# cherise215/advchain

Measured on AMD Instinct MI355X. Metric: augmented images/sec (N adv steps, chain=noise+bias+morph+affine), higher is better.
Workload: dtype f32

## Files before the change

advchain_amd/_lib.py:

```python
import ctypes
import os
from ctypes import c_char_p, c_float, c_int, c_int64, c_void_p

_HERE = os.path.dirname(os.path.abspath(__file__))
LIB_PATH = os.path.join(_HERE, "csrc", "libadvchain_hip.so")

_P, _I, _L, _F = c_void_p, c_int, c_int64, c_float

PROTOTYPES = {
    "advchain_version": (_I, []),
    "advchain_last_error": (c_char_p, []),
    "advchain_set_deterministic": (None, [_I]),
    "advchain_get_deterministic": (_I, []),
    "advchain_grid_sample_fwd": (_I, [_P, _P, _P, _L, _L, _I, _P, _P, _I, _I, _I, _P]),
    "advchain_grid_sample_fwd_ride": (_I, [_P, _P, _P, _P, _P, _L, _L, _I, _P, _P, _I, _I, _I, _I, _P]),
    "advchain_scatter_workspace": (_L, [_L, _I, _P]),
    "advchain_grid_sample_bwd": (_I, [_P, _P, _P, _P, _P, _P, _L, _L, _I, _P, _P, _I, _I, _I, _I, _P]),
    "advchain_det_warp_workspace": (_L, [_L, _L, _I, _P]),
    "advchain_grid_sample_bwd_det": (_I, [_P, _P, _P, _P, _P, _P, _L, _L, _I, _P, _P, _I, _I, _I, _P]),
    "advchain_compose_self_fwd": (_I, [_P, _P, _P, _L, _I, _P, _I, _P, _P]),
    "advchain_compose_self_bwd": (_I, [_P, _P, _P, _P, _I, _I, _L, _I, _P, _P]),
    "advchain_affine_warp_fwd": (_I, [_P, _P, _P, _L, _L, _I, _P, _I, _I, _P]),
    "advchain_affine_warp_fwd_ride": (_I, [_P, _P, _P, _P, _P, _L, _L, _I, _P, _I, _I, _I, _P]),
    "advchain_affine_warp_bwd_workspace": (_L, [_L, _I, _P]),
    "advchain_affine_warp_bwd": (_I, [_P, _P, _P, _P, _P, _P, _L, _L, _I, _P, _I, _I, _P]),
    "advchain_affine_warp_bwd_det": (_I, [_P, _P, _P, _P, _P, _P, _P, _L, _L, _I, _P, _I, _I, _P]),
    "advchain_affine_theta_fwd": (_I, [_P, _P, _F, _P, _P, _L, _I, _P]),
    "advchain_affine_theta_bwd": (_I, [_P, _P, _F, _P, _P, _P, _L, _I, _P]),
    "advchain_tp_interp_fwd": (_I, [_P, _P, _P, _P, _P, _P, _P, _L, _L, _I, _I, _F, _P, _P, _P]),
    "advchain_tp_interp_fwd_smoothed_pair": (_I, [_P, _P, _P, _P, _P, _P, _P, _P, _L, _L, _I, _F, _P, _P, _F, _P]),
    "advchain_band_reduce_axis": (_I, [_P, _P, _P, _P, _P, _P, _P, _P, _I, _L, _L, _F, _P]),
    "advchain_band_reduce_rows_dense": (_I, [_P, _P, _P, _P, _P, _L, _L, _L, _L, _F, _P]),
    "advchain_bias_field_fwd": (_I, [_P, _P, _P, _P, _P, _P, _P, _P, _P, _L, _L, _F, _I, _F, _P]),
    "advchain_bias_field_bwd": (_I, [_P, _P, _P, _P, _P, _P, _P, _P, _P, _P, _L, _L, _F, _I, _F, _P]),
    "advchain_gauss_axis": (_I, [_P, _P, _P, _L, _L, _I, _P, _I, _P, _I, _I, _F, _P]),
    "advchain_gauss_axis_generic": (_I, [_P, _P, _L, _I, _P, _I, _P, _I, _F, _P]),
    "advchain_max_displacement": (_I, [_P, _P, _L, _I, _P, _P]),
    "advchain_grid_sample_bicubic2d_fwd": (_I, [_P, _P, _P, _L, _L, _P, _P, _I, _P]),
    "advchain_grid_sample_bicubic2d_bwd": (_I, [_P, _P, _P, _P, _P, _L, _L, _P, _P, _I, _P]),
    "advchain_affine_grid2d_fwd": (_I, [_P, _P, _L, _P, _P]),
# ... 163 lines not shown
```

advchain_amd/csrc/common.h:

```cpp
#pragma once
#include <hip/hip_runtime.h>
#include <stdint.h>

namespace advchain {

enum { INTERP_LINEAR = 0, INTERP_NEAREST = 1 };
enum { PAD_ZEROS = 0, PAD_BORDER = 1, PAD_REFLECTION = 2 };

constexpr int kBlock = 256;

struct Dims {
  int s0, s1, s2;
  __host__ __device__ int64_t voxels() const { return (int64_t)s0 * s1 * s2; }
};

__device__ __forceinline__ float mul_nc(float a, float b) {
#pragma clang fp contract(off)
  return a * b;
}

__device__ __forceinline__ float lin_coord(int i, int S) {
  if (S <= 1) return S == 1 ? -1.f : 0.f;
  const float step = 2.f / (float)(S - 1);
  return (i < S / 2) ? (-1.f + step * (float)i) : (1.f - step * (float)(S - 1 - i));
// ... 135 lines not shown
__device__ __forceinline__ float fix_out(float cell, const FixScale& s) { return __builtin_amdgcn_ldexpf(cell * s.inv, -s.shift); }
__device__ __forceinline__ bool fix_plain(const FixScale& s, float& scale, float& inv) {
  scale = __builtin_amdgcn_ldexpf(s.mul, s.shift);
  inv = __builtin_amdgcn_ldexpf(s.inv, -s.shift);
  return scale <= 3.40282347e38f && inv >= 1.17549435e-38f && inv <= 3.40282347e38f;
}
__device__ __forceinline__ float fix_out_add(float cell, float a, const FixScale& s) {
  return __builtin_amdgcn_ldexpf(fmaf(cell, s.inv, __builtin_amdgcn_ldexpf(a, s.shift)), -s.shift);
}

__device__ __forceinline__ void atomic_add_f32(float* p, float v) {
  unsafeAtomicAdd(p, v);
}

}

#define ADVCHAIN_OK 0
#define ADVCHAIN_ERR_ARG (-1)
#define ADVCHAIN_ERR_UNSUPPORTED (-2)
#define ADVCHAIN_ERR_LAUNCH (-3)

extern "C" void advchain_set_error_(const char* msg);

#define ADVCHAIN_CHECK_ARG(cond, msg)      \
  do {                                     \
    if (!(cond)) {                         \
      advchain_set_error_(msg);            \
      return ADVCHAIN_ERR_ARG;             \
    }                                      \
  } while (0)

#define ADVCHAIN_LAUNCH_CHECK()                          \
  do {                                                   \
    hipError_t e_ = hipGetLastError();                   \
    if (e_ != hipSuccess) {                              \
      advchain_set_error_(hipGetErrorString(e_));        \
      return ADVCHAIN_ERR_LAUNCH;                        \
    }                                                    \
  } while (0)

static inline int advchain_blocks(int64_t n, int per_block) { return (int)((n + per_block - 1) / per_block); }

static __global__ void __launch_bounds__(256) k_zero_fill(float* __restrict__ p, int64_t n) {
  const int64_t stride = (int64_t)gridDim.x * 256 * 4;
  for (int64_t i = ((int64_t)blockIdx.x * 256 + threadIdx.x) * 4; i < n; i += stride) {
    if (i + 4 <= n && ((uintptr_t)(p + i) & 15) == 0) {
// ... 14 lines not shown
```

advchain_amd/csrc/error.cpp:

```cpp
#include <string.h>

#include <atomic>

static thread_local char g_last_error[512] = "";

extern "C" void advchain_set_error_(const char* msg) {
  strncpy(g_last_error, msg ? msg : "", sizeof(g_last_error) - 1);
  g_last_error[sizeof(g_last_error) - 1] = 0;
}

extern "C" const char* advchain_last_error(void) { return g_last_error; }

static std::atomic<int> g_deterministic{0};
extern "C" void advchain_set_deterministic(int on) { g_deterministic.store(on ? 1 : 0, std::memory_order_relaxed); }
extern "C" int advchain_get_deterministic(void) { return g_deterministic.load(std::memory_order_relaxed); }

extern "C" int advchain_version(void) { return 180; }
```

advchain_amd/csrc/sampler.hip:

```cpp
#include <stdlib.h>
#include "sampler_common.h"
#include "affine_geo.h"
#include "det_fix.h"

namespace advchain {

template <int UNR>
__device__ __forceinline__ void load_str(const float* __restrict__ p, int n, float (&r)[UNR]) {
#pragma unroll
  for (int k = 0; k < UNR; ++k) r[k] = p[(k < n ? k : 0) * kBlock];
#pragma unroll
  for (int k = 0; k < UNR; ++k) r[k] = k < n ? r[k] : 0.f;
}
template <int UNR>
__device__ __forceinline__ void store_str(float* __restrict__ p, int n, const float (&r)[UNR]) {
#pragma unroll
  for (int k = 0; k < UNR; ++k)
    if (k < n) p[k * kBlock] = r[k];
}
__device__ __forceinline__ int active_count(int64_t v0, int64_t total, int unr) {
  if (v0 >= total) return 0;
  const int64_t left = (total - v0 + kBlock - 1) / kBlock;
  return left < unr ? (int)left : unr;
}
// ... 633 lines not shown
}

}

using namespace advchain;

int advchain_scatter_tiled_launch(bool self, const float* gout, const float* in, const float* grid, float* gin,
                                  float* ggrid, int64_t N, int64_t C, int ndim, Dims d, int padding, int clamp_grid,
                                  int32_t* workspace, int chain, int halo, hipStream_t st);

int advchain_self_adjoint_gather_launch(const float* gout, const float* phi, float* gphi, int64_t N, int ndim, Dims d,
                                        int32_t* workspace, int chain, int halo, hipStream_t st);

int advchain_warp_adjoint_gather_launch(const float* gout, const float* in, const float* grid, float* gin, float* ggrid,
                                        int64_t N, int64_t C, int ndim, Dims d, int padding, int clamp_grid,
                                        int32_t* workspace, int halo, hipStream_t st);

int advchain_scatter_march_launch(bool self, const float* gout, const float* in, const float* grid, float* gin, float* ggrid,
                                  int64_t N, int64_t C, Dims d, int padding, int clamp_grid, int H, int32_t* workspace,
                                  hipStream_t st);

int advchain_scatter_window_launch(bool self, const float* gout, const float* in, const float* grid, float* gin,
                                   float* ggrid, int64_t N, int64_t C, int ndim, Dims d, int padding, int clamp_grid,
                                   int halo, int32_t* workspace, hipStream_t st, int32_t* det_ws);
int advchain_scatter_rows2d_launch(bool self, const float* gout, const float* in, const float* grid, float* gin, float* ggrid,
                                   int64_t N, int64_t C, Dims d, int padding, int clamp_grid, int H, int32_t* workspace,
                                   hipStream_t st, int rm_flags = 0);
bool advchain_scatter_rows2d_takes(bool self, int64_t C, Dims d, int padding, int H, int64_t N);

bool advchain_affine_box_fwd_launch(const float* in, const float* theta, float* out, int64_t N, int64_t C, int ndim, Dims d,
                                    hipStream_t st, const float* ride_in = nullptr, float* ride_out = nullptr,
                                    int ride_nonzero = 0);
int advchain_affine_box_tiles(int ndim, Dims d);
int advchain_affine_box_gtheta_launch(const float* gout, const float* in, const float* theta, float* gpart, int64_t N,
                                      int64_t C, int ndim, Dims d, int max_blocks, hipStream_t st, float* tilemax, float* geo = nullptr, int* mode = nullptr);
bool advchain_affine_box_gin_launch(const float* gout, const float* theta, const float* geo, const int* mode, float* gin,
                                    int64_t N, int64_t C, int ndim, Dims d, hipStream_t st, const float* tilemax);

int advchain_expo_fused_fwd2d_launch(const float* phi0, float* fields, int64_t N, advchain::Dims d, int k, int halos,
                                     float* disp_rows, float* fail_flag, hipStream_t stream, bool query = false);
int advchain_adjoint_fused2d_launch(const float* gk, const float* phi0, const float* fields, float* g0, int64_t N, advchain::Dims d,
                                    int k, int32_t* workspace, hipStream_t st);
int advchain_sample_tiled_launch(bool self, const float* in, const float* grid, float* out, const float* phi0,
                                 int64_t N, int64_t C, int ndim, Dims d, int padding, int clamp_grid, int final_mode,
                                 int halo, float* disp_out, hipStream_t st, int disp_hint);

static inline bool use_unroll(int64_t voxels, int ndim) {
// ... 150 lines not shown
}

int advchain_grid_sample_fwd_ride(const float* in, const float* grid, float* out, const float* ride_in, float* ride_out,
                                  int64_t N, int64_t C, int ndim, const int64_t* in_dims, const int64_t* out_dims, int interp,
                                  int padding, int clamp_grid, int flags, void* stream) {
  ADVCHAIN_CHECK_ARG(ride_in && ride_out && ride_out != out, "grid_sample_fwd_ride: null/aliased rider");
  ADVCHAIN_CHECK_ARG((flags & ~1) == 0, "grid_sample_fwd_ride: unknown flags");
  if (ndim == 2 && in && grid && out && dims_ok(ndim, in_dims) && dims_ok(ndim, out_dims, 1) && N > 0 && N < 65536 && C >= 1 &&
      (interp == INTERP_LINEAR || interp == INTERP_NEAREST) && padding >= 0 && padding <= 2) {
    const Dims id = make_dims(ndim, in_dims), od = make_dims(ndim, out_dims);
    ADVCHAIN_CHECK_ARG(id.voxels() < (1ll << 31) && od.voxels() < (1ll << 31), "grid_sample_fwd_ride: per-sample volume too large");
    return launch_grid_sample_fwd<2>(in, grid, out, N, C, id, od, interp, padding, clamp_grid & 1, (hipStream_t)stream, ride_in,
                                     ride_out, flags & 1);
  }
  int rc = advchain_grid_sample_fwd(in, grid, out, N, C, ndim, in_dims, out_dims, interp, padding, clamp_grid, stream);
  if (rc != ADVCHAIN_OK) return rc;
  rc = advchain_grid_sample_fwd(ride_in, grid, ride_out, N, 1, ndim, in_dims, out_dims, interp, padding, clamp_grid, stream);
  if (rc != ADVCHAIN_OK || !(flags & 1) || N == 0) return rc;
  int64_t total = N;
  for (int a = 0; a < ndim; ++a) total *= out_dims[a];
  return advchain_nonzero_mask(ride_out, ride_out, total, stream);
}

int advchain_grid_sample_bwd(const float* grad_out, const float* in, const float* grid, float* grad_in,
                             float* grad_grid, int32_t* workspace, int64_t N, int64_t C, int ndim,
                             const int64_t* in_dims, const int64_t* out_dims, int interp, int padding, int clamp_grid,
                             int halo, void* stream) {
  ADVCHAIN_CHECK_ARG(grad_out && in && grid, "grid_sample_bwd: null pointer");
  ADVCHAIN_CHECK_ARG(grad_in || grad_grid, "grid_sample_bwd: nothing to compute");
  ADVCHAIN_CHECK_ARG(dims_ok(ndim, in_dims) && dims_ok(ndim, out_dims, 1), "grid_sample_bwd: bad dims");
  ADVCHAIN_CHECK_ARG(N >= 0 && N < 65536 && C >= 1, "grid_sample_bwd: bad N/C");
  ADVCHAIN_CHECK_ARG(interp == INTERP_LINEAR || interp == INTERP_NEAREST, "grid_sample_bwd: interp");
  ADVCHAIN_CHECK_ARG(padding >= 0 && padding <= 2, "grid_sample_bwd: padding");
  if (N == 0) return ADVCHAIN_OK;
  const Dims id = make_dims(ndim, in_dims), od = make_dims(ndim, out_dims);
  ADVCHAIN_CHECK_ARG(id.voxels() < (1ll << 31) && od.voxels() < (1ll << 31), "grid_sample_bwd: per-sample volume too large");
  const bool same = id.s0 == od.s0 && id.s1 == od.s1 && id.s2 == od.s2;
  if (workspace && grad_in && same && interp == INTERP_LINEAR && C <= 4) {
    if (ndim == 2 && halo <= -2) {
      const int rr = advchain_scatter_rows2d_launch(false, grad_out, in, grid, grad_in, grad_grid, N, C, id, padding, clamp_grid,
                                                    -halo, workspace, (hipStream_t)stream);
      if (rr != ADVCHAIN_ERR_UNSUPPORTED) return rr;
    }
    const int rc = advchain_warp_adjoint_gather_launch(grad_out, in, grid, grad_in, grad_grid, N, C, ndim, id, padding,
                                                       clamp_grid, workspace, halo, (hipStream_t)stream);
    if (rc != ADVCHAIN_ERR_UNSUPPORTED) return rc;
    if (ndim == 3 && halo <= -2) {
      const int rm = advchain_scatter_march_launch(false, grad_out, in, grid, grad_in, grad_grid, N, C, id, padding, clamp_grid,
                                                   -halo, workspace, (hipStream_t)stream);
      if (rm != ADVCHAIN_ERR_UNSUPPORTED) return rm;
    }
    const int rw = advchain_scatter_window_launch(false, grad_out, in, grid, grad_in, grad_grid, N, C, ndim, id, padding,
                                                  clamp_grid, halo, nullptr, (hipStream_t)stream, workspace);
    if (rw != ADVCHAIN_ERR_UNSUPPORTED) return rw;
    return advchain_scatter_tiled_launch(false, grad_out, in, grid, grad_in, grad_grid, N, C, ndim, id, padding,
                                         clamp_grid, workspace, 0, halo < 0 ? -halo : halo, (hipStream_t)stream);
  }
  if (workspace && grad_in) advchain_zero_async(grad_in, sizeof(float) * N * C * id.voxels(), (hipStream_t)stream);
  return ndim == 3 ? launch_grid_sample_bwd<3>(grad_out, in, grid, grad_in, grad_grid, N, C, id, od, interp, padding, clamp_grid, (hipStream_t)stream)
                   : launch_grid_sample_bwd<2>(grad_out, in, grid, grad_in, grad_grid, N, C, id, od, interp, padding, clamp_grid, (hipStream_t)stream);
}

int64_t advchain_det_warp_workspace(int64_t N, int64_t C, int ndim, const int64_t* in_dims) {
  if (!in_dims || !dims_ok(ndim, in_dims, 1) || N < 0 || C < 1) return -1;
  return det_warp_image_ints(N, C, make_dims(ndim, in_dims).voxels()) + ((N + 3) & ~(int64_t)3);
}

int advchain_grid_sample_bwd_det(const float* grad_out, const float* in, const float* grid, float* grad_in,
                                 float* grad_grid, int32_t* det_ws, int64_t N, int64_t C, int ndim,
                                 const int64_t* in_dims, const int64_t* out_dims, int interp, int padding, int clamp_grid,
                                 void* stream) {
  ADVCHAIN_CHECK_ARG(grad_out && in && grid, "grid_sample_bwd_det: null pointer");
  ADVCHAIN_CHECK_ARG(grad_in || grad_grid, "grid_sample_bwd_det: nothing to compute");
  ADVCHAIN_CHECK_ARG(!grad_in || det_ws, "grid_sample_bwd_det: det_ws required for grad_in (advchain_det_warp_workspace int32 elements)");
  ADVCHAIN_CHECK_ARG(in_dims && out_dims && dims_ok(ndim, in_dims) && dims_ok(ndim, out_dims, 1), "grid_sample_bwd_det: bad dims");
  ADVCHAIN_CHECK_ARG(N >= 0 && N < 65536 && C >= 1, "grid_sample_bwd_det: bad N/C");
  ADVCHAIN_CHECK_ARG(interp == INTERP_LINEAR || interp == INTERP_NEAREST, "grid_sample_bwd_det: interp");
  ADVCHAIN_CHECK_ARG(padding >= 0 && padding <= 2, "grid_sample_bwd_det: padding");
  if (N == 0) return ADVCHAIN_OK;
  const Dims id = make_dims(ndim, in_dims), od = make_dims(ndim, out_dims);
  ADVCHAIN_CHECK_ARG(id.voxels() < (1ll << 31) && od.voxels() < (1ll << 31), "grid_sample_bwd_det: per-sample volume too large");
  hipStream_t st = (hipStream_t)stream;
  clamp_grid &= 1;
// ... 455 lines not shown
```

advchain_amd/csrc/scatter_window.hip:

```cpp
#include <stdlib.h>
#include "sampler_common.h"
#include "det_fix.h"

namespace advchain {

template <bool DET>
__device__ __forceinline__ void win_global_add(float* __restrict__ gin, unsigned long long* __restrict__ acc, int64_t idx,
                                               float v, const FixScale& sdet) {
  if (DET) atomicAdd(acc + idx, (unsigned long long)__float2ll_rn(fix_in(v * sdet.mul, sdet)));
  else atomic_add_f32(gin + idx, v);
}
#ifndef ADVCHAIN_WINDOW_FLAT
#define ADVCHAIN_WINDOW_FLAT 1
#endif
constexpr int kWinT = 32;
constexpr int kWinCells = 8192;
constexpr int kWinCellsC4 = 12288;

template <int PAD, int C, bool SELF, bool GG, bool DET = false>
__global__ void __launch_bounds__(kBlock)
k_scatter_window2d(const float* __restrict__ gout, const float* __restrict__ in, const float* __restrict__ grid,
                   float* __restrict__ gin, float* __restrict__ ggrid, Dims d, int n2, int clamp_grid,
                   int32_t* __restrict__ ws, unsigned long long* __restrict__ acc64 = nullptr,
                   const float* __restrict__ maxn = nullptr) {
  constexpr int kCells2 = C == 4 ? kWinCellsC4 : kWinCells;
  __shared__ int win[kCells2];
  if (ws && blockIdx.x == 0 && blockIdx.y == 0 && threadIdx.x == 0) ws[3] = -1;
  __shared__ int red[8][kBlock / 64];
  constexpr int DIM = 2;
  constexpr int SPT = kWinT * kWinT / kBlock;
  const int V = (int)d.voxels();
  const int n = blockIdx.y;
  const int tx = blockIdx.x % n2, ty = blockIdx.x / n2;
  const int lx = threadIdx.x & 31, ly0 = threadIdx.x >> 5;
  const int sx = tx * kWinT + lx;
  const float* gn = grid + (int64_t)n * DIM * V;
  const float* gon = gout + (int64_t)n * C * V;
  const float* inn = in + (int64_t)n * C * V;
  float* ginn = gin + (int64_t)n * C * V;
  unsigned long long* accn = DET ? acc64 + (int64_t)n * C * V : nullptr;
  const FixScale sdet = DET ? det_scale(maxn, n) : FixScale{0, 0.f, 0.f};

  Taps<DIM, PAD> t[SPT];
  float go[SPT][C];
  bool live[SPT], px[SPT], py[SPT];
  int bx0 = 1 << 30, bx1 = -(1 << 30), by0 = 1 << 30, by1 = -(1 << 30);
  float gmax = 0.f;
#pragma unroll
  for (int j = 0; j < SPT; ++j) {
    const int sy = ty * kWinT + ly0 + 8 * j;
    live[j] = sx < d.s2 && sy < d.s1;
    const int s = live[j] ? sy * d.s2 + sx : 0;
    float gx = gn[s], gy = gn[V + s];
    px[j] = py[j] = true;
    if (clamp_grid) {
      px[j] = gx >= -1.f && gx <= 1.f; py[j] = gy >= -1.f && gy <= 1.f;
      gx = clamp_unit(gx); gy = clamp_unit(gy);
    }
    t[j].build(gx, gy, 0.f, d);
#pragma unroll
    for (int c = 0; c < C; ++c) {
      const float g = gon[(int64_t)c * V + s];
      go[j][c] = live[j] ? g : 0.f;
      gmax = fmaxf(gmax, fabsf(go[j][c]));
    }
    if (live[j]) {
      if (t[j].x.v0 || t[j].x.v1) { bx0 = min(bx0, t[j].x.i0 + (t[j].x.v0 ? 0 : 1)); bx1 = max(bx1, t[j].x.i0 + (t[j].x.v1 ? 1 : 0)); }
      if (t[j].y.v0 || t[j].y.v1) { by0 = min(by0, t[j].y.i0 + (t[j].y.v0 ? 0 : 1)); by1 = max(by1, t[j].y.i0 + (t[j].y.v1 ? 1 : 0)); }
    }
  }
#pragma unroll
  for (int o = 32; o > 0; o >>= 1) {
    bx0 = min(bx0, __shfl_xor(bx0, o, 64)); bx1 = max(bx1, __shfl_xor(bx1, o, 64));
    by0 = min(by0, __shfl_xor(by0, o, 64)); by1 = max(by1, __shfl_xor(by1, o, 64));
    gmax = fmaxf(gmax, __shfl_xor(gmax, o, 64));
  }
  const int wave = threadIdx.x >> 6;
  if ((threadIdx.x & 63) == 0) {
    red[0][wave] = bx0; red[1][wave] = bx1; red[2][wave] = by0; red[3][wave] = by1; red[4][wave] = __float_as_int(gmax);
  }
  __syncthreads();
#pragma unroll
  for (int w = 0; w < kBlock / 64; ++w) {
    bx0 = min(bx0, red[0][w]); bx1 = max(bx1, red[1][w]); by0 = min(by0, red[2][w]); by1 = max(by1, red[3][w]);
    gmax = fmaxf(gmax, __int_as_float(red[4][w]));
  }
  int ww = max(bx1 - bx0 + 1, 0), wh = max(by1 - by0 + 1, 0);
  constexpr int cells_per_ch = kCells2 / C;
  if (ww > 128) ww = 128;
  if (ww > 0 && wh > cells_per_ch / ww) wh = cells_per_ch / ww;
  const int cells = ww * wh;
  for (int i = threadIdx.x; i < C * cells; i += kBlock) win[i] = 0;
  const FixScale fs = fix_scale(gmax, 20);
  __syncthreads();

  float cgx[SPT], cgy[SPT];
  if (SELF || GG) {
#pragma unroll
    for (int j = 0; j < SPT; ++j) {
      float ax = 0.f, ay = 0.f, dummy = 0.f;
#pragma unroll
      for (int c = 0; c < C; ++c)
        sample_linear_bwd<DIM, PAD, false, true>(inn + (int64_t)c * V, nullptr, go[j][c], t[j], d, ax, ay, dummy);
      cgx[j] = px[j] ? t[j].x.mult * ax : 0.f;
      cgy[j] = py[j] ? t[j].y.mult * ay : 0.f;
    }
  }

#pragma unroll
  for (int j = 0; j < SPT; ++j) {
    if (!live[j]) continue;
    const int sy = ty * kWinT + ly0 + 8 * j;
    const int s = sy * d.s2 + sx;
    const int wx0 = t[j].x.i0 - bx0, wy0 = t[j].y.i0 - by0;
    const int cell0 = __mul24(wy0, ww) + wx0;
    const int vox0 = __mul24(t[j].y.i0, d.s2) + t[j].x.i0;
    const bool inx[2] = {wx0 >= 0 && wx0 < ww, wx0 + 1 >= 0 && wx0 + 1 < ww};
    const bool iny[2] = {wy0 >= 0 && wy0 < wh, wy0 + 1 >= 0 && wy0 + 1 < wh};
#pragma unroll
    for (int cy = 0; cy < 2; ++cy)
#pragma unroll
      for (int cx = 0; cx < 2; ++cx) {
        if (!t[j].ok(0, cy, cx)) continue;
        const float w = t[j].w(0, cy, cx);
        if (inx[cx] && iny[cy]) {
          const float ws = w * fs.mul;
          int* cell = win + cell0 + (cy ? ww : 0) + cx;
#pragma unroll
          for (int c = 0; c < C; ++c) atomicAdd(cell + c * cells, fix_round(ws * fix_in(go[j][c], fs)));
        } else {
          const int64_t dst = vox0 + (cy ? d.s2 : 0) + cx;
#pragma unroll
          for (int c = 0; c < C; ++c) win_global_add<DET>(ginn, accn, dst + (int64_t)c * V, w * go[j][c], sdet);
        }
      }
    if (SELF || GG) {
      const float ggx = cgx[j], ggy = cgy[j];
      if (SELF) {
        if (ggx != 0.f) win_global_add<DET>(ginn, accn, s, ggx, sdet);
        if (ggy != 0.f) win_global_add<DET>(ginn, accn, (int64_t)V + s, ggy, sdet);
      } else {
        float* gg = ggrid + (int64_t)n * DIM * V + s;
        gg[0] = ggx;
        gg[V] = ggy;
      }
    }
  }
  __syncthreads();

  for (int i = threadIdx.x; i < C * cells; i += kBlock) {
    const int a = win[i];
    if (a == 0) continue;
    const int c = i / cells, r = i - c * cells;
    const int wy = r / ww, wx = r - wy * ww;
    win_global_add<DET>(ginn, accn, (int64_t)c * V + (by0 + wy) * d.s2 + (bx0 + wx), fix_out((float)a, fs), sdet);
  }
}

#ifndef ADVCHAIN_WIN3_CP4
#define ADVCHAIN_WIN3_CP4 2
#endif
#ifndef ADVCHAIN_WIN3_CPS
#define ADVCHAIN_WIN3_CPS 3
#endif
constexpr int kWin3CP4 = ADVCHAIN_WIN3_CP4, kWin3CPS = ADVCHAIN_WIN3_CPS;
constexpr int kWin3Cells = 12288;

template <int PAD, int C, bool SELF, bool GG, int TX, int TZ, bool DET = false>
__global__ void __launch_bounds__(kBlock)
k_scatter_window3d(const float* __restrict__ gout, const float* __restrict__ in, const float* __restrict__ grid,
                   float* __restrict__ gin, float* __restrict__ ggrid, Dims d, int n1, int n2, int clamp_grid,
                   int32_t* __restrict__ ws, unsigned long long* __restrict__ acc64 = nullptr,
                   const float* __restrict__ maxn = nullptr) {
  __shared__ int win[kWin3Cells];
  constexpr int CP = C == 4 ? kWin3CP4 : (SELF ? kWin3CPS : C);
  if (ws && blockIdx.x == 0 && blockIdx.y == 0 && threadIdx.x == 0) ws[3] = -1;
  __shared__ int red[7][kBlock / 64];
  constexpr int DIM = 3;
// ... 184 lines not shown
  {
    const float inv_ww = 1.f / (float)max(ww, 1), inv_wh = 1.f / (float)max(wh, 1), inv_wd = 1.f / (float)max(wd, 1);
    for (int i = threadIdx.x; i < CP * cells; i += kBlock) {
      const int a = win[i];
      if (a == 0) continue;
      const int r = (int)(((float)i + 0.5f) * inv_ww), wx = i - r * ww;
      const int rz = (int)(((float)r + 0.5f) * inv_wh), wy = r - rz * wh;
      const int c = (int)(((float)rz + 0.5f) * inv_wd), wz = rz - c * wd;
      win_global_add<DET>(ginn, accn, (int64_t)(c0 + c) * V + ((lo[2] + wz) * d.s1 + (lo[1] + wy)) * d.s2 + (lo[0] + wx),
                          fix_out((float)a, fs), sdet);
    }
  }
  if (c0 + CP < C) __syncthreads();
  }
}

}

using namespace advchain;

extern "C" int advchain_get_deterministic(void);
int advchain_scatter_window_launch(bool self, const float* gout, const float* in, const float* grid, float* gin,
                                   float* ggrid, int64_t N, int64_t C, int ndim, Dims d, int padding, int clamp_grid,
                                   int halo, int32_t* workspace, hipStream_t st, int32_t* det_ws) {
  static const bool off = getenv("ADVCHAIN_NO_WINDOW_SCATTER") != nullptr;
  static const int min3 = 2;
  if (off || padding == PAD_REFLECTION) return ADVCHAIN_ERR_UNSUPPORTED;
  if (d.s2 >= (1 << 23) || (int64_t)d.s0 * d.s1 >= (1 << 23)) return ADVCHAIN_ERR_UNSUPPORTED;
  if (self ? C != ndim : (C != 1 && C != 2 && C != 4)) return ADVCHAIN_ERR_UNSUPPORTED;
  if (ndim == 3 && (halo < 0 ? -halo : halo) < min3) return ADVCHAIN_ERR_UNSUPPORTED;
  const bool det = advchain_get_deterministic() != 0 && det_ws != nullptr;
  const int64_t V = d.voxels();
  unsigned long long* acc64 = nullptr;
  float* maxn = nullptr;
  if (det) {
    acc64 = reinterpret_cast<unsigned long long*>(det_ws + 4 + 2 * N * V);
    maxn = reinterpret_cast<float*>(det_ws + 4 + 2 * N * V + 8 * N * V);
    advchain_zero_async(acc64, sizeof(unsigned long long) * N * C * V, st);
    advchain_zero_async(maxn, sizeof(float) * N, st);
    const int64_t per_n = C * V;
    int64_t nb = (per_n + kBlock * 16 - 1) / (kBlock * 16);
    if (nb > 1024) nb = 1024;
    hipLaunchKernelGGL(k_det_absmax, dim3((unsigned)nb, (unsigned)N), dim3(kBlock), 0, st, gout, maxn, per_n);
  } else {
    advchain_zero_async(gin, sizeof(float) * N * C * V, st);
  }
  const bool gg = ggrid != nullptr;
  dim3 b(kBlock);
#define GO_PAD(C_, SELF_, GG_) \
  do { if (padding == PAD_BORDER) GO(PAD_BORDER, C_, SELF_, GG_); else GO(PAD_ZEROS, C_, SELF_, GG_); } while (0)
#define GO_ALL(CS_) \
  do { \
    if (self) GO(PAD_BORDER, CS_, true, false); \
    else if (C == 1) { if (gg) GO_PAD(1, false, true); else GO_PAD(1, false, false); } \
    else if (C == 2) { if (gg) GO_PAD(2, false, true); else GO_PAD(2, false, false); } \
// ... 16 lines not shown
    const int n2 = (d.s2 + TXs - 1) / TXs, n1 = (d.s1 + TYs - 1) / TYs, n0 = (d.s0 + TZs - 1) / TZs;
    dim3 g((unsigned)(n0 * n1 * n2), (unsigned)N);
#define GO3(PAD_, C_, SELF_, GG_, TX_, DET_) \
  hipLaunchKernelGGL((k_scatter_window3d<PAD_, C_, SELF_, GG_, TX_, 4, DET_>), g, b, 0, st, gout, in, grid, gin, ggrid, d, n1, n2, clamp_grid, workspace, acc64, maxn)
#define GO(PAD_, C_, SELF_, GG_) \
  do { \
    if (sh == 0) { if (det) GO3(PAD_, C_, SELF_, GG_, 32, true); else GO3(PAD_, C_, SELF_, GG_, 32, false); } \
    else { if (det) GO3(PAD_, C_, SELF_, GG_, 16, true); else GO3(PAD_, C_, SELF_, GG_, 16, false); } \
  } while (0)
    GO_ALL(3);
#undef GO
#undef GO3
  }
#undef GO_ALL
#undef GO_PAD
  if (det) {
    const int64_t per_n = C * V;
    int64_t nb = (per_n + kBlock * 8 - 1) / (kBlock * 8);
    if (nb > 2048) nb = 2048;
    hipLaunchKernelGGL(k_det_convert, dim3((unsigned)nb, (unsigned)N), dim3(kBlock), 0, st, reinterpret_cast<const long long*>(acc64),
                       maxn, gin, per_n);
  }
  ADVCHAIN_LAUNCH_CHECK();
  return ADVCHAIN_OK;
}
```

advchain_amd/ops.py:

```python
import ctypes
import functools
import os

import numpy as np
import torch

from . import _lib
from .bands import gaussian_weights_1d

_INTERP = {"bilinear": 0, "trilinear": 0, "linear": 0, "nearest": 1, "bicubic": 2}
_PAD = {"zeros": 0, "border": 1, "reflection": 2}
_GAUSS9 = _lib.float_array(gaussian_weights_1d(1.0))
_GAUSS9_CACHE = {}


GENERIC_MAX_TAPS = 129


def gauss9(sigma, taps=None):
    sigma = float(sigma)
    if taps is None:
        taps = 2 * int(4 * sigma + 0.5) + 1
    taps = int(taps)
    if sigma == 1.0 and taps == 9:
# ... 118 lines not shown
    N, C = inp.shape[:2]
    nd = inp.dim() - 2
    odims = tuple(grid.shape[2:])
    out = torch.empty((N, C) + odims, device=inp.device, dtype=torch.float32)
    rout = torch.empty((N, 1) + odims, device=inp.device, dtype=torch.float32)
    _lib.check(_lib.load().advchain_grid_sample_fwd_ride(_ptr(inp), _ptr(grid), _ptr(out), _ptr(ride), _ptr(rout), N, C, nd,
                                                         _lib.dims_array(inp.shape[2:]), _lib.dims_array(odims), interp, padding,
                                                         int(clamp_grid) | _hint_bits(disp_hint), int(bool(nonzero)), _stream()),
               "grid_sample_fwd_ride")
    return out, rout


DISP_SLOTS = 4096
ADAPTIVE_HALO = os.environ.get("ADVCHAIN_NO_ADAPTIVE_HALO") is None
PAIR_FIELDS = os.environ.get("ADVCHAIN_NO_PAIR_FIELDS") is None
TILED_SCATTER = True
FUSED_LOSS = True
WIDE_LOSS_MIN_K = 17
REF_GRAD_REG_MAX_K = 4
FUSE_2D = True
COMPOSITE = True
RIDE_MASK = True
RIDE_INTERPS = ("bilinear", "trilinear", "linear", "nearest")


def set_deterministic(on):
    _lib.load().advchain_set_deterministic(1 if on else 0)


def is_deterministic():
    return bool(_lib.load().advchain_get_deterministic())


def _scatter_workspace(N, dims, device):
    n = _lib.load().advchain_scatter_workspace(N, len(dims), _lib.dims_array(dims))
    return torch.empty(n, device=device, dtype=torch.int32)


def _det_warp_workspace(N, C, dims, device):
    n = _lib.load().advchain_det_warp_workspace(N, C, len(dims), _lib.dims_array(dims))
    return torch.empty(max(1, n), device=device, dtype=torch.int32)


def _general_warp_kernel(C, interp, in_dims, out_dims):
    return C > 4 or interp != 0 or tuple(in_dims) != tuple(out_dims)


def raw_grid_sample_bwd(gout, inp, grid, interp, padding, clamp_grid, need_gin, need_ggrid, halo=0):
    N, C = inp.shape[:2]
    nd = inp.dim() - 2
    if need_gin and is_deterministic() and _general_warp_kernel(C, interp, inp.shape[2:], grid.shape[2:]):
        ws = _det_warp_workspace(N, C, inp.shape[2:], inp.device)
        gin = torch.empty_like(inp)
        ggrid = torch.empty_like(grid) if need_ggrid else None
        _lib.check(_lib.load().advchain_grid_sample_bwd_det(_ptr(gout), _ptr(inp), _ptr(grid), _ptr(gin), _ptr(ggrid), _ptr(ws),
                                                            N, C, nd, _lib.dims_array(inp.shape[2:]),
                                                            _lib.dims_array(grid.shape[2:]), interp, padding, int(clamp_grid),
                                                            _stream()), "grid_sample_bwd_det")
        return gin, ggrid
    tiled = TILED_SCATTER and need_gin
    ws = _scatter_workspace(N, inp.shape[2:], inp.device) if tiled else None
    gin = (torch.empty_like(inp) if tiled else torch.zeros_like(inp)) if need_gin else None
    ggrid = torch.empty_like(grid) if need_ggrid else None
    _lib.check(_lib.load().advchain_grid_sample_bwd(_ptr(gout), _ptr(inp), _ptr(grid), _ptr(gin), _ptr(ggrid), _ptr(ws),
                                                    N, C, nd, _lib.dims_array(inp.shape[2:]),
                                                    _lib.dims_array(grid.shape[2:]), interp, padding, int(clamp_grid),
                                                    int(halo), _stream()), "grid_sample_bwd")
    return gin, ggrid


def raw_compose_self_fwd(phi, phi0=None, final_mode=0, disp_out=None, disp_hint=None):
    N = phi.shape[0]
    nd = phi.dim() - 2
    out = torch.empty_like(phi)
    _lib.check(_lib.load().advchain_compose_self_fwd(_ptr(phi), _ptr(out), _ptr(phi0), N, nd,
                                                     _lib.dims_array(phi.shape[2:]), final_mode | _hint_bits(disp_hint), _ptr(disp_out),
                                                     _stream()), "compose_self_fwd")
    return out


def raw_compose_self_bwd(gout, phi, ws=None, chain=False, halo=0):
    N = phi.shape[0]
    nd = phi.dim() - 2
    if TILED_SCATTER and ws is None:
        ws, chain = _scatter_workspace(N, phi.shape[2:], phi.device), False
    gphi = torch.empty_like(phi) if ws is not None else torch.zeros_like(phi)
# ... 1781 lines not shown
```

include/advchain_hip.h:

```cpp
#ifndef ADVCHAIN_HIP_H_
#define ADVCHAIN_HIP_H_

#include <stdint.h>

#ifdef __cplusplus
extern "C" {
#endif

#define ADVCHAIN_INTERP_LINEAR 0
#define ADVCHAIN_INTERP_NEAREST 1
#define ADVCHAIN_INTERP_BICUBIC 2
#define ADVCHAIN_PAD_ZEROS 0
#define ADVCHAIN_PAD_BORDER 1
#define ADVCHAIN_PAD_REFLECTION 2

int advchain_version(void);
const char* advchain_last_error(void);

void advchain_set_deterministic(int on);
int advchain_get_deterministic(void);

int advchain_grid_sample_fwd(const float* in, const float* grid, float* out, int64_t N, int64_t C, int ndim,
                             const int64_t* in_dims, const int64_t* out_dims, int interp, int padding,
                             int clamp_grid, void* stream);
int advchain_grid_sample_fwd_ride(const float* in, const float* grid, float* out, const float* ride_in, float* ride_out,
                                  int64_t N, int64_t C, int ndim, const int64_t* in_dims, const int64_t* out_dims,
                                  int interp, int padding, int clamp_grid, int flags, void* stream);
int64_t advchain_scatter_workspace(int64_t N, int ndim, const int64_t* dims);
int advchain_grid_sample_bwd(const float* grad_out, const float* in, const float* grid, float* grad_in,
                             float* grad_grid, int32_t* workspace, int64_t N, int64_t C, int ndim,
                             const int64_t* in_dims, const int64_t* out_dims, int interp, int padding, int clamp_grid,
                             int halo, void* stream);
int64_t advchain_det_warp_workspace(int64_t N, int64_t C, int ndim, const int64_t* in_dims);
int advchain_grid_sample_bwd_det(const float* grad_out, const float* in, const float* grid, float* grad_in,
                                 float* grad_grid, int32_t* det_ws, int64_t N, int64_t C, int ndim,
                                 const int64_t* in_dims, const int64_t* out_dims, int interp, int padding, int clamp_grid,
                                 void* stream);

#define ADVCHAIN_DISP_SLOTS 4096
int advchain_compose_self_fwd(const float* phi, float* out, const float* phi0, int64_t N, int ndim,
                              const int64_t* dims, int final_mode, float* disp_out, void* stream);
int advchain_compose_self_bwd(const float* grad_out, const float* phi, float* grad_phi, int32_t* workspace, int chain,
                              int halo, int64_t N, int ndim, const int64_t* dims, void* stream);
int advchain_expo_chain_fused_levels(int64_t N, int ndim, const int64_t* dims, int n, const int32_t* hints);
int advchain_expo_chain_fwd(const float* phi0, float* fields, float* pos, int64_t N, int ndim, const int64_t* dims, int n,
                            float* disp_rows, const int32_t* hints, float* fuse_flag, void* stream);
int advchain_expo_chain_bwd(const float* grad_pos, const float* phi0, const float* fields, float* grad_phi0, float* scratch,
                            int32_t* workspace, const int32_t* halos, int64_t N, int ndim, const int64_t* dims, int n,
                            void* stream);
int advchain_demons_compose_pair_fwd(const float* vel, float* s1, float* phi0, float* fields, float* pos, float* q,
                                     float* disp, float* rows_max, const int32_t* itab, const float* ftab,
                                     const int64_t* S3, const int64_t* g3, const int64_t* B3, int64_t N, int ndim, int n,
                                     const int32_t* hints, const float* weights9_host, float scale, float inv, int fuse,
                                     void* stream);
int advchain_demons_compose_pair_bwd(const float* gq_lo, const float* gq_hi, const float* pos, const float* phi0,
// ... 216 lines not shown
```

Measured before the change: 4252.

## Add staged two-pass window scatter for deterministic 2D warp backward

In deterministic mode, 2D warp backward with 1, 2 or 4 channels now has each tile dump its shared-memory fixed-point window and a header to a staging buffer. A second merge kernel then gathers, for each output tile, all overlapping staged windows and sums them in int64 before writing grad_in. This replaces global 64-bit atomics and the separate max-norm pass of the old deterministic path. The cost is a large staging buffer, an extra kernel, and a merge that scans every tile header per output tile. A thread-local route tracker is also added for introspection.

Result: faster. 4338 (median of 6 runs) (+2.0%).

```diff
diff --git a/advchain_amd/_lib.py b/advchain_amd/_lib.py
--- a/advchain_amd/_lib.py
+++ b/advchain_amd/_lib.py
@@ -16,6 +16,9 @@
     "advchain_grid_sample_fwd_ride": (_I, [_P, _P, _P, _P, _P, _L, _L, _I, _P, _P, _I, _I, _I, _I, _P]),
     "advchain_scatter_workspace": (_L, [_L, _I, _P]),
     "advchain_grid_sample_bwd": (_I, [_P, _P, _P, _P, _P, _P, _L, _L, _I, _P, _P, _I, _I, _I, _I, _P]),
+    "advchain_window_stage_workspace": (_L, [_L, _L, _I, _P]),
+    "advchain_grid_sample_bwd_staged": (_I, [_P, _P, _P, _P, _P, _P, _L, _L, _I, _P, _P, _I, _I, _I, _I, _P, _P]),
+    "advchain_last_bwd_route": (_I, []),
     "advchain_det_warp_workspace": (_L, [_L, _L, _I, _P]),
     "advchain_grid_sample_bwd_det": (_I, [_P, _P, _P, _P, _P, _P, _L, _L, _I, _P, _P, _I, _I, _I, _P]),
     "advchain_compose_self_fwd": (_I, [_P, _P, _P, _L, _I, _P, _I, _P, _P]),
diff --git a/advchain_amd/csrc/common.h b/advchain_amd/csrc/common.h
--- a/advchain_amd/csrc/common.h
+++ b/advchain_amd/csrc/common.h
@@ -181,6 +181,17 @@
 
 extern "C" void advchain_set_error_(const char* msg);
 
+#define ADVCHAIN_ROUTE_NONE 0
+#define ADVCHAIN_ROUTE_GENERAL 1
+#define ADVCHAIN_ROUTE_ROWS 2
+#define ADVCHAIN_ROUTE_GATHER 3
+#define ADVCHAIN_ROUTE_MARCH 4
+#define ADVCHAIN_ROUTE_WINDOW_FLOAT 5
+#define ADVCHAIN_ROUTE_WINDOW_INT64 6
+#define ADVCHAIN_ROUTE_WINDOW_STAGED 7
+#define ADVCHAIN_ROUTE_TILED 8
+extern "C" void advchain_set_route_(int route);
+
 #define ADVCHAIN_CHECK_ARG(cond, msg)      \
   do {                                     \
     if (!(cond)) {                         \
diff --git a/advchain_amd/csrc/error.cpp b/advchain_amd/csrc/error.cpp
--- a/advchain_amd/csrc/error.cpp
+++ b/advchain_amd/csrc/error.cpp
@@ -15,4 +15,8 @@
 extern "C" void advchain_set_deterministic(int on) { g_deterministic.store(on ? 1 : 0, std::memory_order_relaxed); }
 extern "C" int advchain_get_deterministic(void) { return g_deterministic.load(std::memory_order_relaxed); }
 
-extern "C" int advchain_version(void) { return 180; }
+static thread_local int g_last_bwd_route = 0;
+extern "C" void advchain_set_route_(int route) { g_last_bwd_route = route; }
+extern "C" int advchain_last_bwd_route(void) { return g_last_bwd_route; }
+
+extern "C" int advchain_version(void) { return 190; }
diff --git a/advchain_amd/csrc/sampler.hip b/advchain_amd/csrc/sampler.hip
--- a/advchain_amd/csrc/sampler.hip
+++ b/advchain_amd/csrc/sampler.hip
@@ -679,7 +679,8 @@
 
 int advchain_scatter_window_launch(bool self, const float* gout, const float* in, const float* grid, float* gin,
                                    float* ggrid, int64_t N, int64_t C, int ndim, Dims d, int padding, int clamp_grid,
-                                   int halo, int32_t* workspace, hipStream_t st, int32_t* det_ws);
+                                   int halo, int32_t* workspace, hipStream_t st, int32_t* det_ws, int32_t* stage_ws = nullptr);
+int64_t advchain_window_stage_ints(int64_t N, int64_t C, Dims d);
 int advchain_scatter_rows2d_launch(bool self, const float* gout, const float* in, const float* grid, float* gin, float* ggrid,
                                    int64_t N, int64_t C, Dims d, int padding, int clamp_grid, int H, int32_t* workspace,
                                    hipStream_t st, int rm_flags = 0);
@@ -876,10 +877,10 @@
   return advchain_nonzero_mask(ride_out, ride_out, total, stream);
 }
 
-int advchain_grid_sample_bwd(const float* grad_out, const float* in, const float* grid, float* grad_in,
-                             float* grad_grid, int32_t* workspace, int64_t N, int64_t C, int ndim,
-                             const int64_t* in_dims, const int64_t* out_dims, int interp, int padding, int clamp_grid,
-                             int halo, void* stream) {
+static int grid_sample_bwd_routed(const float* grad_out, const float* in, const float* grid, float* grad_in,
+                                  float* grad_grid, int32_t* workspace, int64_t N, int64_t C, int ndim,
+                                  const int64_t* in_dims, const int64_t* out_dims, int interp, int padding, int clamp_grid,
+                                  int halo, void* stream, int32_t* stage_ws) {
   ADVCHAIN_CHECK_ARG(grad_out && in && grid, "grid_sample_bwd: null pointer");
   ADVCHAIN_CHECK_ARG(grad_in || grad_grid, "grid_sample_bwd: nothing to compute");
   ADVCHAIN_CHECK_ARG(dims_ok(ndim, in_dims) && dims_ok(ndim, out_dims, 1), "grid_sample_bwd: bad dims");
@@ -894,25 +895,53 @@
     if (ndim == 2 && halo <= -2) {
       const int rr = advchain_scatter_rows2d_launch(false, grad_out, in, grid, grad_in, grad_grid, N, C, id, padding, clamp_grid,
                                                     -halo, workspace, (hipStream_t)stream);
-      if (rr != ADVCHAIN_ERR_UNSUPPORTED) return rr;
+      if (rr != ADVCHAIN_ERR_UNSUPPORTED) { advchain_set_route_(ADVCHAIN_ROUTE_ROWS); return rr; }
     }
     const int rc = advchain_warp_adjoint_gather_launch(grad_out, in, grid, grad_in, grad_grid, N, C, ndim, id, padding,
                                                        clamp_grid, workspace, halo, (hipStream_t)stream);
-    if (rc != ADVCHAIN_ERR_UNSUPPORTED) return rc;
+    if (rc != ADVCHAIN_ERR_UNSUPPORTED) { advchain_set_route_(ADVCHAIN_ROUTE_GATHER); return rc; }
     if (ndim == 3 && halo <= -2) {
       const int rm = advchain_scatter_march_launch(false, grad_out, in, grid, grad_in, grad_grid, N, C, id, padding, clamp_grid,
                                                    -halo, workspace, (hipStream_t)stream);
-      if (rm != ADVCHAIN_ERR_UNSUPPORTED) return rm;
+      if (rm != ADVCHAIN_ERR_UNSUPPORTED) { advchain_set_route_(ADVCHAIN_ROUTE_MARCH); return rm; }
     }
     const int rw = advchain_scatter_window_launch(false, grad_out, in, grid, grad_in, grad_grid, N, C, ndim, id, padding,
-                                                  clamp_grid, halo, nullptr, (hipStream_t)stream, workspace);
+                                                  clamp_grid, halo, nullptr, (hipStream_t)stream, workspace, stage_ws);
     if (rw != ADVCHAIN_ERR_UNSUPPORTED) return rw;
+    advchain_set_route_(ADVCHAIN_ROUTE_TILED);
     return advchain_scatter_tiled_launch(false, grad_out, in, grid, grad_in, grad_grid, N, C, ndim, id, padding,
                                          clamp_grid, workspace, 0, halo < 0 ? -halo : halo, (hipStream_t)stream);
   }
   if (workspace && grad_in) advchain_zero_async(grad_in, sizeof(float) * N * C * id.voxels(), (hipStream_t)stream);
+  advchain_set_route_(ADVCHAIN_ROUTE_GENERAL);
   return ndim == 3 ? launch_grid_sample_bwd<3>(grad_out, in, grid, grad_in, grad_grid, N, C, id, od, interp, padding, clamp_grid, (hipStream_t)stream)
                    : launch_grid_sample_bwd<2>(grad_out, in, grid, grad_in, grad_grid, N, C, id, od, interp, padding, clamp_grid, (hipStream_t)stream);
+}
+
+int advchain_grid_sample_bwd(const float* grad_out, const float* in, const float* grid, float* grad_in,
+                             float* grad_grid, int32_t* workspace, int64_t N, int64_t C, int ndim,
+                             const int64_t* in_dims, const int64_t* out_dims, int interp, int padding, int clamp_grid,
+                             int halo, void* stream) {
+  return grid_sample_bwd_routed(grad_out, in, grid, grad_in, grad_grid, workspace, N, C, ndim, in_dims, out_dims, interp, padding,
+                                clamp_grid, halo, stream, nullptr);
+}
+
+int64_t advchain_window_stage_workspace(int64_t N, int64_t C, int ndim, const int64_t* dims) {
+  if (!dims || !dims_ok(ndim, dims) || N < 0 || N >= 65536 || C < 1) return -1;
+  if (ndim != 2 || (C != 1 && C != 2 && C != 4)) return 0;
+  return advchain_window_stage_ints(N, C, make_dims(ndim, dims));
+}
+
+int advchain_grid_sample_bwd_staged(const float* grad_out, const float* in, const float* grid, float* grad_in,
+                                    float* grad_grid, int32_t* workspace, int64_t N, int64_t C, int ndim,
+                                    const int64_t* in_dims, const int64_t* out_dims, int interp, int padding, int clamp_grid,
+                                    int halo, void* stream, int32_t* stage_ws) {
+  ADVCHAIN_CHECK_ARG(!stage_ws || (workspace && grad_in), "grid_sample_bwd_staged: stage_ws needs workspace and grad_in");
+  ADVCHAIN_CHECK_ARG(!stage_ws || (((uintptr_t)stage_ws) & 15) == 0, "grid_sample_bwd_staged: stage_ws must be 16-byte aligned");
+  ADVCHAIN_CHECK_ARG(!stage_ws || (ndim == 2 && (C == 1 || C == 2 || C == 4)),
+                     "grid_sample_bwd_staged: stage_ws is for 2D warps of 1, 2 or 4 channels (advchain_window_stage_workspace)");
+  return grid_sample_bwd_routed(grad_out, in, grid, grad_in, grad_grid, workspace, N, C, ndim, in_dims, out_dims, interp, padding,
+                                clamp_grid, halo, stream, stage_ws);
 }
 
 int64_t advchain_det_warp_workspace(int64_t N, int64_t C, int ndim, const int64_t* in_dims) {
diff --git a/advchain_amd/csrc/scatter_window.hip b/advchain_amd/csrc/scatter_window.hip
--- a/advchain_amd/csrc/scatter_window.hip
+++ b/advchain_amd/csrc/scatter_window.hip
@@ -17,12 +17,20 @@
 constexpr int kWinCells = 8192;
 constexpr int kWinCellsC4 = 12288;
 
-template <int PAD, int C, bool SELF, bool GG, bool DET = false>
+constexpr int kWinHead = 8;
+struct WinStage {
+  int32_t* head;
+  int32_t* cells;
+};
+__device__ __forceinline__ WinStage win_stage_of(const WinStage& s) { return s; }
+
+template <int PAD, int C, bool SELF, bool GG, bool DET = false, class... STG>
 __global__ void __launch_bounds__(kBlock)
 k_scatter_window2d(const float* __restrict__ gout, const float* __restrict__ in, const float* __restrict__ grid,
                    float* __restrict__ gin, float* __restrict__ ggrid, Dims d, int n2, int clamp_grid,
                    int32_t* __restrict__ ws, unsigned long long* __restrict__ acc64 = nullptr,
-                   const float* __restrict__ maxn = nullptr) {
+                   const float* __restrict__ maxn = nullptr, STG... stg) {
+  constexpr bool STAGE = sizeof...(STG) > 0;
   constexpr int kCells2 = C == 4 ? kWinCellsC4 : kWinCells;
   __shared__ int win[kCells2];
   if (ws && blockIdx.x == 0 && blockIdx.y == 0 && threadIdx.x == 0) ws[3] = -1;
@@ -46,6 +54,7 @@
   bool live[SPT], px[SPT], py[SPT];
   int bx0 = 1 << 30, bx1 = -(1 << 30), by0 = 1 << 30, by1 = -(1 << 30);
   float gmax = 0.f;
+  bool bad = false, outside = false;
 #pragma unroll
   for (int j = 0; j < SPT; ++j) {
     const int sy = ty * kWinT + ly0 + 8 * j;
@@ -63,6 +72,7 @@
       const float g = gon[(int64_t)c * V + s];
       go[j][c] = live[j] ? g : 0.f;
       gmax = fmaxf(gmax, fabsf(go[j][c]));
+      if constexpr (STAGE) bad = bad || !(fabsf(go[j][c]) <= 3.0e38f);
     }
     if (live[j]) {
       if (t[j].x.v0 || t[j].x.v1) { bx0 = min(bx0, t[j].x.i0 + (t[j].x.v0 ? 0 : 1)); bx1 = max(bx1, t[j].x.i0 + (t[j].x.v1 ? 1 : 0)); }
@@ -79,11 +89,16 @@
   if ((threadIdx.x & 63) == 0) {
     red[0][wave] = bx0; red[1][wave] = bx1; red[2][wave] = by0; red[3][wave] = by1; red[4][wave] = __float_as_int(gmax);
   }
+  if constexpr (STAGE) {
+    const bool wave_bad = __ballot(bad) != 0;
+    if ((threadIdx.x & 63) == 0) red[5][wave] = wave_bad;
+  }
   __syncthreads();
 #pragma unroll
   for (int w = 0; w < kBlock / 64; ++w) {
     bx0 = min(bx0, red[0][w]); bx1 = max(bx1, red[1][w]); by0 = min(by0, red[2][w]); by1 = max(by1, red[3][w]);
     gmax = fmaxf(gmax, __int_as_float(red[4][w]));
+    if constexpr (STAGE) bad = bad || red[5][w] != 0;
   }
   int ww = max(bx1 - bx0 + 1, 0), wh = max(by1 - by0 + 1, 0);
   constexpr int cells_per_ch = kCells2 / C;
@@ -128,6 +143,8 @@
           int* cell = win + cell0 + (cy ? ww : 0) + cx;
 #pragma unroll
           for (int c = 0; c < C; ++c) atomicAdd(cell + c * cells, fix_round(ws * fix_in(go[j][c], fs)));
+        } else if constexpr (STAGE) {
+          outside = true;
         } else {
           const int64_t dst = vox0 + (cy ? d.s2 : 0) + cx;
 #pragma unroll
@@ -146,7 +163,26 @@
       }
     }
   }
+  if constexpr (STAGE) {
+    const bool wave_out = __ballot(outside) != 0;
+    if ((threadIdx.x & 63) == 0) red[6][wave] = wave_out;
+  }
   __syncthreads();
+
+  if constexpr (STAGE) {
+    const WinStage sg = win_stage_of(stg...);
+    const int64_t slot = (int64_t)n * gridDim.x + blockIdx.x;
+    int32_t* sc = sg.cells + slot * kCells2;
+    for (int i = threadIdx.x; i < C * cells; i += kBlock) sc[i] = win[i];
+    if (threadIdx.x == 0) {
+      int flags = bad ? 1 : 0;
+#pragma unroll
+      for (int w = 0; w < kBlock / 64; ++w) flags |= red[6][w] != 0 ? 2 : 0;
+      int32_t* h = sg.head + slot * kWinHead;
+      h[0] = bx0; h[1] = by0; h[2] = ww; h[3] = wh; h[4] = bx1; h[5] = by1; h[6] = __float_as_int(gmax); h[7] = flags;
+    }
+    return;
+  }
 
   for (int i = threadIdx.x; i < C * cells; i += kBlock) {
     const int a = win[i];
@@ -154,6 +190,148 @@
     const int c = i / cells, r = i - c * cells;
     const int wy = r / ww, wx = r - wy * ww;
     win_global_add<DET>(ginn, accn, (int64_t)c * V + (by0 + wy) * d.s2 + (bx0 + wx), fix_out((float)a, fs), sdet);
+  }
+}
+
+template <int PAD, int C>
+__global__ void __launch_bounds__(kBlock)
+k_window_merge2d(const float* __restrict__ gout, const float* __restrict__ grid, float* __restrict__ gin, Dims d, int n2,
+                 int clamp_grid, WinStage sg) {
+  constexpr int kCells2 = C == 4 ? kWinCellsC4 : kWinCells;
+  constexpr int SPT = kWinT * kWinT / kBlock;
+  __shared__ unsigned long long cap[C * kWinT * kWinT];
+  __shared__ int list[kBlock][kWinHead];
+  __shared__ int nlist;
+  __shared__ float wm[kBlock / 64];
+  const int V = (int)d.voxels();
+  const int T = gridDim.x, n = blockIdx.y;
+  const int rx0 = (blockIdx.x % n2) * kWinT, ry0 = (blockIdx.x / n2) * kWinT;
+  const int lx = threadIdx.x & 31, ly0 = threadIdx.x >> 5;
+  const int px = rx0 + lx;
+  const int32_t* hn = sg.head + (int64_t)n * T * kWinHead;
+  const int32_t* cn = sg.cells + (int64_t)n * T * kCells2;
+  const float* gn = grid + (int64_t)n * 2 * V;
+  const float* gon = gout + (int64_t)n * C * V;
+
+  float m = 0.f;
+  bool bad = false;
+  for (int t = threadIdx.x; t < T; t += kBlock) {
+    m = fmaxf(m, __int_as_float(hn[t * kWinHead + 6]));
+    bad = bad || (hn[t * kWinHead + 7] & 1) != 0;
+  }
+  if (bad) m = __int_as_float(0x7f800000);
+#pragma unroll
+  for (int o = 32; o > 0; o >>= 1) m = fmaxf(m, __shfl_xor(m, o, 64));
+  if ((threadIdx.x & 63) == 0) wm[threadIdx.x >> 6] = m;
+  __syncthreads();
+#pragma unroll
+  for (int w = 0; w < kBlock / 64; ++w) m = fmaxf(m, wm[w]);
+  const FixScale sdet = fix_scale(m, kDetBits);
+
+  long long sum[SPT][C];
+#pragma unroll
+  for (int j = 0; j < SPT; ++j)
+#pragma unroll
+    for (int c = 0; c < C; ++c) sum[j][c] = 0;
+  bool used_cap = false;
+
+  for (int t0 = 0; t0 < T; t0 += kBlock) {
+    __syncthreads();
+    if (threadIdx.x == 0) nlist = 0;
+    __syncthreads();
+    if (t0 + (int)threadIdx.x < T) {
+      const int t = t0 + threadIdx.x;
+      const int4 a = *reinterpret_cast<const int4*>(hn + t * kWinHead), b = *reinterpret_cast<const int4*>(hn + t * kWinHead + 4);
+      const int bx0 = a.x, by0 = a.y, ww = a.z, wh = a.w, bx1 = b.x, by1 = b.y;
+      const bool meets = ww > 0 && wh > 0 && bx0 < rx0 + kWinT && bx0 + ww > rx0 && by0 < ry0 + kWinT && by0 + wh > ry0;
+      const bool walk = (b.w & 2) != 0 && bx0 < rx0 + kWinT && bx1 >= rx0 && by0 < ry0 + kWinT && by1 >= ry0;
+      if (meets || walk) {
+        int* e = list[atomicAdd(&nlist, 1)];
+        e[0] = bx0; e[1] = by0; e[2] = ww; e[3] = wh; e[4] = b.z; e[5] = t; e[6] = (meets ? 1 : 0) | (walk ? 2 : 0);
+      }
+    }
+    __syncthreads();
+    const int nl = nlist;
+    for (int k = 0; k < nl; ++k) {
+      const int bx0 = list[k][0], by0 = list[k][1], ww = list[k][2], wh = list[k][3], tile = list[k][5], what = list[k][6];
+      if (what & 1) {
+        const FixScale fs = fix_scale(__int_as_float(list[k][4]), 20);
+        const int32_t* sc = cn + (int64_t)tile * kCells2;
+        const int cells = ww * wh;
+        const int wx = px - bx0;
+        const bool okx = wx >= 0 && wx < ww;
+        int a[SPT][C];
+#pragma unroll
+        for (int j = 0; j < SPT; ++j) {
+          const int wy = ry0 + ly0 + 8 * j - by0;
+          const bool ok = okx && wy >= 0 && wy < wh;
+          const int cell = ok ? wy * ww + wx : 0;
+#pragma unroll
+          for (int c = 0; c < C; ++c) {
+            const int v = sc[c * cells + cell];
+            a[j][c] = ok ? v : 0;
+          }
+        }
+#pragma unroll
+        for (int j = 0; j < SPT; ++j)
+#pragma unroll
+          for (int c = 0; c < C; ++c) {
+            const long long q = __float2ll_rn(fix_in(fix_out((float)a[j][c], fs) * sdet.mul, sdet));
+            sum[j][c] += a[j][c] != 0 ? q : 0ll;
+          }
+      }
+      if (what & 2) {
+        if (!used_cap) {
+          for (int i = threadIdx.x; i < C * kWinT * kWinT; i += kBlock) cap[i] = 0ull;
+          used_cap = true;
+          __syncthreads();
+        }
+        const int sx = (tile % n2) * kWinT + lx;
+#pragma unroll
+        for (int j = 0; j < SPT; ++j) {
+          const int sy = (tile / n2) * kWinT + ly0 + 8 * j;
+          if (!(sx < d.s2 && sy < d.s1)) continue;
+          const int s = sy * d.s2 + sx;
+          float gx = gn[s], gy = gn[V + s];
+          if (clamp_grid) { gx = clamp_unit(gx); gy = clamp_unit(gy); }
+          Taps<2, PAD> t;
+          t.build(gx, gy, 0.f, d);
+          float go[C];
+#pragma unroll
+          for (int c = 0; c < C; ++c) go[c] = gon[(int64_t)c * V + s];
+          const int wx0 = t.x.i0 - bx0, wy0 = t.y.i0 - by0;
+          const bool inx[2] = {wx0 >= 0 && wx0 < ww, wx0 + 1 >= 0 && wx0 + 1 < ww};
+          const bool iny[2] = {wy0 >= 0 && wy0 < wh, wy0 + 1 >= 0 && wy0 + 1 < wh};
+#pragma unroll
+          for (int cy = 0; cy < 2; ++cy)
+#pragma unroll
+            for (int cx = 0; cx < 2; ++cx) {
+              if (!t.ok(0, cy, cx) || (inx[cx] && iny[cy])) continue;
+              const int qx = t.x.i0 + cx - rx0, qy = t.y.i0 + cy - ry0;
+              if (qx < 0 || qx >= kWinT || qy < 0 || qy >= kWinT) continue;
+              const float w = t.w(0, cy, cx);
+#pragma unroll
+              for (int c = 0; c < C; ++c)
+                atomicAdd(cap + c * kWinT * kWinT + qy * kWinT + qx,
+                          (unsigned long long)__float2ll_rn(fix_in((w * go[c]) * sdet.mul, sdet)));
+            }
+        }
+      }
+    }
+  }
+  if (used_cap) __syncthreads();
+
+  float* ginn = gin + (int64_t)n * C * V;
+#pragma unroll
+  for (int j = 0; j < SPT; ++j) {
+    const int py = ry0 + ly0 + 8 * j;
+    if (!(px < d.s2 && py < d.s1)) continue;
+#pragma unroll
+    for (int c = 0; c < C; ++c) {
+      long long q = sum[j][c];
+      if (used_cap) q += (long long)cap[c * kWinT * kWinT + (ly0 + 8 * j) * kWinT + lx];
+      ginn[(int64_t)c * V + py * d.s2 + px] = fix_out((float)q, sdet);
+    }
   }
 }
 
@@ -384,7 +562,7 @@
 extern "C" int advchain_get_deterministic(void);
 int advchain_scatter_window_launch(bool self, const float* gout, const float* in, const float* grid, float* gin,
                                    float* ggrid, int64_t N, int64_t C, int ndim, Dims d, int padding, int clamp_grid,
-                                   int halo, int32_t* workspace, hipStream_t st, int32_t* det_ws) {
+                                   int halo, int32_t* workspace, hipStream_t st, int32_t* det_ws, int32_t* stage_ws) {
   static const bool off = getenv("ADVCHAIN_NO_WINDOW_SCATTER") != nullptr;
   static const int min3 = 2;
   if (off || padding == PAD_REFLECTION) return ADVCHAIN_ERR_UNSUPPORTED;
@@ -393,6 +571,28 @@
   if (ndim == 3 && (halo < 0 ? -halo : halo) < min3) return ADVCHAIN_ERR_UNSUPPORTED;
   const bool det = advchain_get_deterministic() != 0 && det_ws != nullptr;
   const int64_t V = d.voxels();
+  if (det && !self && ndim == 2 && stage_ws != nullptr) {
+    const int n2 = (d.s2 + kWinT - 1) / kWinT, n1 = (d.s1 + kWinT - 1) / kWinT;
+    const int64_t tiles = (int64_t)n1 * n2;
+    const WinStage sg{stage_ws, stage_ws + N * tiles * kWinHead};
+    const dim3 g((unsigned)tiles, (unsigned)N), b(kBlock);
+    unsigned long long* const no_acc = nullptr;
+    const float* const no_max = nullptr;
+#define GO_ST(PAD_, C_) \
+  do { \
+    if (ggrid) hipLaunchKernelGGL((k_scatter_window2d<PAD_, C_, false, true, false, WinStage>), g, b, 0, st, gout, in, grid, gin, ggrid, d, n2, clamp_grid, workspace, no_acc, no_max, sg); \
+    else hipLaunchKernelGGL((k_scatter_window2d<PAD_, C_, false, false, false, WinStage>), g, b, 0, st, gout, in, grid, gin, ggrid, d, n2, clamp_grid, workspace, no_acc, no_max, sg); \
+    hipLaunchKernelGGL((k_window_merge2d<PAD_, C_>), g, b, 0, st, gout, grid, gin, d, n2, clamp_grid, sg); \
+  } while (0)
+#define GO_STC(PAD_) \
+  do { if (C == 1) GO_ST(PAD_, 1); else if (C == 2) GO_ST(PAD_, 2); else GO_ST(PAD_, 4); } while (0)
+    if (padding == PAD_BORDER) GO_STC(PAD_BORDER); else GO_STC(PAD_ZEROS);
+#undef GO_STC
+#undef GO_ST
+    ADVCHAIN_LAUNCH_CHECK();
+    advchain_set_route_(ADVCHAIN_ROUTE_WINDOW_STAGED);
+    return ADVCHAIN_OK;
+  }
   unsigned long long* acc64 = nullptr;
   float* maxn = nullptr;
   if (det) {
@@ -455,5 +655,11 @@
                        maxn, gin, per_n);
   }
   ADVCHAIN_LAUNCH_CHECK();
+  advchain_set_route_(det ? ADVCHAIN_ROUTE_WINDOW_INT64 : ADVCHAIN_ROUTE_WINDOW_FLOAT);
   return ADVCHAIN_OK;
 }
+
+int64_t advchain_window_stage_ints(int64_t N, int64_t C, Dims d) {
+  const int64_t tiles = (int64_t)((d.s2 + kWinT - 1) / kWinT) * ((d.s1 + kWinT - 1) / kWinT);
+  return N * tiles * ((C == 4 ? kWinCellsC4 : kWinCells) + kWinHead);
+}
diff --git a/advchain_amd/ops.py b/advchain_amd/ops.py
--- a/advchain_amd/ops.py
+++ b/advchain_amd/ops.py
@@ -164,6 +164,14 @@
 COMPOSITE = True
 RIDE_MASK = True
 RIDE_INTERPS = ("bilinear", "trilinear", "linear", "nearest")
+WINDOW_STAGED = True
+WINDOW_STAGED_CHANNELS = (1, 2, 4)
+
+BWD_ROUTES = ("none", "general", "rows", "gather", "march", "window_float", "window_int64", "window_staged", "tiled")
+
+
+def last_bwd_route():
+    return BWD_ROUTES[_lib.load().advchain_last_bwd_route()]
 
 
 def set_deterministic(on):
@@ -204,6 +212,16 @@
     ws = _scatter_workspace(N, inp.shape[2:], inp.device) if tiled else None
     gin = (torch.empty_like(inp) if tiled else torch.zeros_like(inp)) if need_gin else None
     ggrid = torch.empty_like(grid) if need_ggrid else None
+    if (tiled and WINDOW_STAGED and nd == 2 and C in WINDOW_STAGED_CHANNELS and is_deterministic()
+            and not _general_warp_kernel(C, interp, inp.shape[2:], grid.shape[2:])):
+        lib = _lib.load()
+        n = lib.advchain_window_stage_workspace(N, C, nd, _lib.dims_array(inp.shape[2:]))
+        stage = torch.empty(max(4, n), device=inp.device, dtype=torch.int32)
+        _lib.check(lib.advchain_grid_sample_bwd_staged(_ptr(gout), _ptr(inp), _ptr(grid), _ptr(gin), _ptr(ggrid), _ptr(ws),
+                                                       N, C, nd, _lib.dims_array(inp.shape[2:]),
+                                                       _lib.dims_array(grid.shape[2:]), interp, padding, int(clamp_grid),
+                                                       int(halo), _stream(), _ptr(stage)), "grid_sample_bwd_staged")
+        return gin, ggrid
     _lib.check(_lib.load().advchain_grid_sample_bwd(_ptr(gout), _ptr(inp), _ptr(grid), _ptr(gin), _ptr(ggrid), _ptr(ws),
                                                     N, C, nd, _lib.dims_array(inp.shape[2:]),
                                                     _lib.dims_array(grid.shape[2:]), interp, padding, int(clamp_grid),
diff --git a/include/advchain_hip.h b/include/advchain_hip.h
--- a/include/advchain_hip.h
+++ b/include/advchain_hip.h
@@ -31,6 +31,21 @@
                              float* grad_grid, int32_t* workspace, int64_t N, int64_t C, int ndim,
                              const int64_t* in_dims, const int64_t* out_dims, int interp, int padding, int clamp_grid,
                              int halo, void* stream);
+int64_t advchain_window_stage_workspace(int64_t N, int64_t C, int ndim, const int64_t* in_dims);
+int advchain_grid_sample_bwd_staged(const float* grad_out, const float* in, const float* grid, float* grad_in,
+                                    float* grad_grid, int32_t* workspace, int64_t N, int64_t C, int ndim,
+                                    const int64_t* in_dims, const int64_t* out_dims, int interp, int padding, int clamp_grid,
+                                    int halo, void* stream, int32_t* stage_ws);
+#define ADVCHAIN_ROUTE_NONE 0
+#define ADVCHAIN_ROUTE_GENERAL 1
+#define ADVCHAIN_ROUTE_ROWS 2
+#define ADVCHAIN_ROUTE_GATHER 3
+#define ADVCHAIN_ROUTE_MARCH 4
+#define ADVCHAIN_ROUTE_WINDOW_FLOAT 5
+#define ADVCHAIN_ROUTE_WINDOW_INT64 6
+#define ADVCHAIN_ROUTE_WINDOW_STAGED 7
+#define ADVCHAIN_ROUTE_TILED 8
+int advchain_last_bwd_route(void);
 int64_t advchain_det_warp_workspace(int64_t N, int64_t C, int ndim, const int64_t* in_dims);
 int advchain_grid_sample_bwd_det(const float* grad_out, const float* in, const float* grid, float* grad_in,
                                  float* grad_grid, int32_t* det_ws, int64_t N, int64_t C, int ndim,
```
